# papaboo/Bifrost3D

Measured on AMD Instinct MI355X. Metric: Mrays/sec + ms/frame at 1080p/256spp; per-pixel RMSE vs OptiXRenderer, higher is better.
Workload: dtype f32

## Files before the change

bifrost3d_amd/csrc/hiprenderer.hip:

```cpp
#include "kernels.h"
#ifndef HIPR_WIDE8_LOW_BUCKET
#define HIPR_WIDE8_LOW_BUCKET 0
#endif
#include "wide8_kernels.h"
#include "wide8_refit.h"
#include "launch.h"

#include <hip/hip_runtime.h>

#include <algorithm>
#include <cmath>
#include <cstdarg>
#include <cstdio>
#include <cstdlib>
#include <cstring>
#include <memory>
#include <string>
#include <vector>

using namespace hipr;

namespace {

thread_local std::string g_last_error;

int fail(int status, const char* fmt, ...) {
    char buf[512];
    va_list args;
    va_start(args, fmt);
    vsnprintf(buf, sizeof(buf), fmt, args);
    va_end(args);
    g_last_error = buf;
    fprintf(stderr, "hiprenderer: %s\n", buf);
    return status;
}

#define HIP_TRY(call)                                                                                          \
    do {                                                                                                       \
        hipError_t err__ = (call);                                                                             \
        if (err__ != hipSuccess)                                                                               \
            return fail(err__ == hipErrorOutOfMemory ? HIPR_ERROR_OUT_OF_MEMORY : HIPR_ERROR_HIP, "%s failed: %s (%s:%d)", #call, \
                        hipGetErrorString(err__), __FILE__, __LINE__);                                         \
    } while (0)

struct DeviceBuffer {
    void* ptr = nullptr;
    size_t bytes = 0;
    DeviceBuffer() = default;
    DeviceBuffer(DeviceBuffer&& other) noexcept : ptr(other.ptr), bytes(other.bytes) { other.ptr = nullptr; other.bytes = 0; }
    DeviceBuffer& operator=(DeviceBuffer&& other) noexcept { std::swap(ptr, other.ptr); std::swap(bytes, other.bytes); return *this; }
    ~DeviceBuffer() { release(); }
    int resize(size_t new_bytes) {
        if (new_bytes <= bytes && ptr) return HIPR_OK;
        if (ptr) { (void)hipFree(ptr); ptr = nullptr; bytes = 0; }
        if (new_bytes == 0) return HIPR_OK;
        HIP_TRY(hipMalloc(&ptr, new_bytes));
        bytes = new_bytes;
        return HIPR_OK;
    }
    int upload(const void* src, size_t n, hipStream_t stream) {
        if (n == 0) return HIPR_OK;
        if (int s = resize(n)) return s;
        HIP_TRY(hipMemcpyAsync(ptr, src, n, hipMemcpyHostToDevice, stream));
        return HIPR_OK;
    }
    void release() { if (ptr) (void)hipFree(ptr); ptr = nullptr; bytes = 0; }
    template <typename T> T* as() const { return static_cast<T*>(ptr); }
};

template <typename T, hipError_t (*FREE)(T)>
struct Owned {
    T handle = nullptr;
    Owned() = default;
    Owned(Owned&& other) noexcept : handle(other.handle) { other.handle = nullptr; }
    Owned& operator=(Owned&& other) noexcept { std::swap(handle, other.handle); return *this; }
    ~Owned() { if (handle) (void)FREE(handle); }
    operator T() const { return handle; }
};
hipError_t free_pinned_words(uint32_t* words) { return hipHostFree(words); }
using Stream = Owned<hipStream_t, hipStreamDestroy>;
using Event = Owned<hipEvent_t, hipEventDestroy>;
using PinnedWords = Owned<uint32_t*, free_pinned_words>;
Stream make_stream() { Stream s; if (hipStreamCreateWithFlags(&s.handle, hipStreamNonBlocking) != hipSuccess) s.handle = nullptr; return s; }
Event make_event(unsigned flags = hipEventDisableTiming) { Event e; if (hipEventCreateWithFlags(&e.handle, flags) != hipSuccess) e.handle = nullptr; return e; }
PinnedWords make_pinned_words(size_t count) { PinnedWords p; if (hipHostMalloc((void**)&p.handle, count * sizeof(uint32_t)) != hipSuccess) p.handle = nullptr; return p; }

struct TimedLaunch { int kernel; hipEvent_t start, stop; };

struct Wavefront {
    Stream own_stream;
    hipStream_t stream = nullptr;
    Event shade_done[2], counts_copied[2], finished;
    DeviceBuffer path[2][4], hits, shadow[3], queue_counts, order, order_coat, nee_flags, sort_keys[2], sort_order, sort_temp;
    PinnedWords host_counts;
    uint32_t first_slot = 0, n_slots = 0;

    PathState path_state(int which) const {
        return {path[which][0].as<float4>(), path[which][1].as<float4>(), path[which][2].as<float4>(), path[which][3].as<uint2>()};
    }
    ShadowQueue shadow_queue() const { return {shadow[0].as<float4>(), shadow[1].as<float4>(), shadow[2].as<float4>()}; }
};
constexpr int MAX_WAVEFRONTS = 4;
constexpr int COUNT_PAIR_STRIDE = 16;
constexpr int COUNT_PAIRS = 3, COUNT_LINES = 5;
constexpr int HOST_COUNT_WORDS = 8 + COUNT_LINES * COUNT_PAIR_STRIDE;

struct Preflight {
    uint32_t wide_stack_need = 0;
    uint32_t wide8_height = 0;
};

struct ResidentScene {
    DeviceBuffer nodes, wide_nodes, wide8_slots, triangles, instances, lights;
    DeviceBuffer indices, geometry, texcoords, tints, emissions, materials, textures, texels, environment_PDF, environment_samples;
    DeviceBuffer shade_triangles, trace_triangles, trace_items;
    DeviceBuffer triangle_class;
    DeviceScene args = {};
    Wide8Scene wide8 = {};
    uint32_t wide8_height = 0, wide_stack_entries = 0;
    int stack_size = 16;
    int shading_models = 7;
    bool coverage_textures_r8 = false;
    bool has_environment = true;
    bool has_textures = true;
    bool all_triangles_opaque = false;
    bool any_coated_triangle = false;
    std::vector<HiprMaterial> uploaded_materials;
    std::vector<uint32_t> uploaded_light_types;
    std::vector<HiprInstance> uploaded_instances;
    uint32_t uploaded_texture_count = 0, uploaded_vertex_count = 0, uploaded_index_count = 0;
    uint64_t uploaded_texel_bytes = 0;

    DeviceBuffer refit_leaf_slots, refit_node_slots, refit_exact, refit_moved, refit_partial, refit_scratch;
    std::vector<uint32_t> refit_level_begin;
    uint32_t refit_leaf_count = 0;
    std::vector<uint32_t> refit_node_list, refit_node_words;
    double uploaded_half_area = 0.0, current_half_area = 0.0;
    bool tree_stale = false;

    bool ready = false;
    int chosen_variant = HIPR_TRACE_BVH2;
    void choose_variant(int requested) {
        const bool large = args.node_count > 64;
        int v = requested;
        if (v < 0) v = large ? HIPR_TRACE_WIDE8_PERSISTENT : (args.triangle_count <= SMALL_SCENE_TRIANGLES ? HIPR_TRACE_EXHAUSTIVE : HIPR_TRACE_BVH2);
        if (v == HIPR_TRACE_WIDE8_PERSISTENT && wide8.slot_count == 0) v = HIPR_TRACE_WIDE_PERSISTENT;
        if (v == HIPR_TRACE_WIDE_PERSISTENT && args.wide_node_count == 0) v = HIPR_TRACE_BVH2;
        if (v == HIPR_TRACE_EXHAUSTIVE && args.trace_item_count == 0 && args.triangle_count != 0) v = HIPR_TRACE_BVH2;
        chosen_variant = v;
    }

    int upload(const HiprSceneDesc* s, const Preflight& checked, int requested_variant, bool cull_backfaces, hipStream_t stream);
    int update_geometry(const HiprSceneDesc* s, const Preflight& checked, int requested_variant, bool cull_backfaces, hipStream_t stream);
    int refit_transforms(const HiprInstanceTransform* moved, uint32_t moved_count, const HiprLight* new_lights, uint32_t light_count, hipStream_t stream, HiprRefitResult* out);
    int lights_keep_their_types(const char* who, const HiprLight* new_lights, uint32_t count) const;
// ... 109 lines not shown
        for (Chain& ch : chains) if (ch.stream == on) return ch;
        for (Chain& ch : chains) if (!ch.event) { ch.stream = on; return ch; }
        chains[0] = {on, nullptr};
        return chains[0];
    }
    void break_chain(hipStream_t on) { chain_of(on).event = nullptr; }
    void begin_timed(int kernel, hipStream_t on) {
        if (!timing) return;
        Chain& ch = chain_of(on);
        TimedLaunch t = {kernel, ch.event ? ch.event : next_event(), next_event()};
        if (!t.start || !t.stop) return;
        if (!ch.event) (void)hipEventRecord(t.start, on);
        ch.event = nullptr;
        timed.push_back(t);
    }
    hipEvent_t end_timed(hipStream_t on) {
        if (!timing || timed.empty()) return nullptr;
        (void)hipEventRecord(timed.back().stop, on);
        chain_of(on).event = timed.back().stop;
        return timed.back().stop;
    }
    void collect_times() {
        for (const TimedLaunch& t : timed) {
            float ms = 0;
            if (hipEventElapsedTime(&ms, t.start, t.stop) == hipSuccess) {
                times.milliseconds[t.kernel] += ms;
                times.launches[t.kernel] += 1;
            }
        }
        timed.clear();
        events_used = 0;
        for (Chain& ch : chains) ch.event = nullptr;
    }
};

namespace {

uint32_t grid_for(uint32_t items, uint32_t block, uint32_t max_blocks) {
    uint32_t blocks = (items + block - 1) / block;
    blocks = std::max(1u, std::min(blocks, max_blocks));
    return (blocks + 7u) & ~7u;
}

constexpr uint32_t PAIRING_LIMIT = SMALL_SCENE_TRIANGLES;
void build_trace_items(const HiprTriangle* triangles, uint32_t count, std::vector<float>& items) {
    auto corner = [&](uint32_t t, int k) -> const float* { const HiprTriangle& tri = triangles[t]; return k % 3 == 0 ? tri.v0 : (k % 3 == 1 ? tri.v1 : tri.v2); };
    auto same = [](const float* p, const float* q) { return std::memcmp(p, q, 12) == 0; };
    auto bits = [](uint32_t v) { float f; std::memcpy(&f, &v, 4); return f; };
    std::vector<bool> merged(count, false);
    items.clear();
    for (uint32_t i = 0; i < count; ++i) {
        if (merged[i]) continue;
        int ra = 0, rb = 0;
        uint32_t partner = UINT32_MAX;
        for (uint32_t j = i + 1; count <= PAIRING_LIMIT && j < count && partner == UINT32_MAX; ++j) {
            if (merged[j] || triangles[j].instance_index != triangles[i].instance_index || triangles[j].flags != triangles[i].flags) continue;
            for (int x = 0; x < 3 && partner == UINT32_MAX; ++x)
                for (int y = 0; y < 3 && partner == UINT32_MAX; ++y) {
                    const float *a = corner(i, x), *b = corner(i, x + 1), *c = corner(i, x + 2), *a2 = corner(j, y), *c2 = corner(j, y + 1), *d = corner(j, y + 2);
                    if (!same(a, a2) || !same(c, c2)) continue;
                    float longest = 0.0f, off = 0.0f;
                    for (int k = 0; k < 3; ++k) {
                        longest = std::fmax(longest, std::fmax(std::fabs(b[k] - a[k]), std::fabs(d[k] - a[k])));
                        off = std::fmax(off, std::fabs(d[k] - (a[k] + (c[k] - b[k]))));
                    }
                    if (off <= 1e-6f * longest) { partner = j; ra = x; rb = y; }
                }
        }
        const float *a = corner(i, ra), *b = corner(i, ra + 1), *d = partner == UINT32_MAX ? corner(i, ra + 2) : corner(partner, rb + 2);
        const uint32_t selectors = partner == UINT32_MAX ? 0u : uint32_t((4 - ra) % 3) | uint32_t((5 - ra) % 3) << 2 | uint32_t((4 - rb) % 3) << 4 | uint32_t((5 - rb) % 3) << 6;
        const float item[16] = {a[0], a[1], a[2], b[0] - a[0], b[1] - a[1], b[2] - a[2], d[0] - a[0], d[1] - a[1], d[2] - a[2],
                                bits(triangles[i].instance_index), bits(triangles[i].primitive_index), bits(triangles[i].flags | (partner == UINT32_MAX ? 0u : HIPR_ITEM_QUAD)),
                                bits(i), bits(partner == UINT32_MAX ? i : partner), bits(partner == UINT32_MAX ? triangles[i].primitive_index : triangles[partner].primitive_index),
                                bits(selectors)};
        items.insert(items.end(), item, item + 16);
        if (partner != UINT32_MAX) merged[partner] = true;
    }
}

constexpr uint32_t WORK_SETS = 256;
constexpr uint32_t WORK_SET_WORDS = TRACE_SHARDS * TRACE_SHARD_STRIDE;
constexpr uint32_t WORK_COUNTERS = WORK_SETS * WORK_SET_WORDS;

uint32_t* next_work_counter(HiprContext* c) {
    uint32_t& index = c->pass_slots[c->active_slot].work_index;
    uint32_t* ring = c->work_counters.as<uint32_t>() + size_t(c->active_slot) * WORK_COUNTERS;
    if (index >= WORK_SETS) {
        for (int g = 0; g < MAX_WAVEFRONTS; ++g) if (c->wavefronts[g].stream) (void)hipStreamSynchronize(c->wavefronts[g].stream);
        (void)hipMemsetAsync(ring, 0, WORK_COUNTERS * sizeof(uint32_t), c->stream);
        (void)hipStreamSynchronize(c->stream);
        index = 0;
    }
    return ring + size_t(index++) * WORK_SET_WORDS;
}

template <int STACK, int MODE, bool INSTRUMENT, bool OVERFLOW>
void launch_persistent(HiprContext* c, const Wavefront& w, const PathState& in, const uint32_t* closest_count, const uint32_t* shadow_count, uint32_t upper_bound, int bucket) {
    int& per_cu = c->persistent_blocks_per_cu[MODE][bucket];
    if (per_cu == 0) {
        int blocks = 0;
        if (hipOccupancyMaxActiveBlocksPerMultiprocessor(&blocks, k_trace_persistent<STACK, MODE, INSTRUMENT, OVERFLOW>, TRACE_BLOCK, 0) != hipSuccess || blocks <= 0) blocks = 4;
        if (c->trace_log) fprintf(stderr, "[hipr] k_trace_persistent<%d, %d>: occupancy query says %d blocks of %d threads per CU\n", STACK, MODE, blocks, TRACE_BLOCK);
        if (c->blocks_per_cu_override > 0) blocks = c->blocks_per_cu_override;
        per_cu = blocks;
    }
    const uint32_t waves_per_block = TRACE_BLOCK / 64;
    uint32_t grid = uint32_t(c->cu_count) * uint32_t(per_cu);
    grid = std::max(1u, std::min(grid, (upper_bound + 63u) / 64u / waves_per_block + 1u));
    hipLaunchKernelGGL((k_trace_persistent<STACK, MODE, INSTRUMENT, OVERFLOW>), dim3(grid), dim3(TRACE_BLOCK), 0, w.stream, c->scene.args, in, w.hits.as<float4>(), w.shadow_queue(),
                       c->radiance.as<float4>(), closest_count, shadow_count, next_work_counter(c), c->refill_below, c->counters.as<DeviceCounters>());
}

template <int STACK, int MODE, bool INSTRUMENT>
void launch_wide8(HiprContext* c, const Wavefront& w, const PathState& in, const uint32_t* closest_count, const uint32_t* shadow_count, uint32_t upper_bound, int bucket, const uint32_t* sorted = nullptr) {
    int& per_cu = c->wide8_blocks_per_cu[MODE][bucket];
    if (per_cu == 0) {
        int blocks = 0;
        if (hipOccupancyMaxActiveBlocksPerMultiprocessor(&blocks, k_trace_wide8<STACK, MODE, INSTRUMENT>, TRACE_BLOCK, 0) != hipSuccess || blocks <= 0) blocks = 4;
        if (c->trace_log) fprintf(stderr, "[hipr] k_trace_wide8<%d, %d>: occupancy query says %d blocks of %d threads per CU\n", STACK, MODE, blocks, TRACE_BLOCK);
        if (c->blocks_per_cu_override > 0) blocks = c->blocks_per_cu_override;
        per_cu = blocks;
    }
    const uint32_t waves_per_block = TRACE_BLOCK / 64;
    uint32_t grid = uint32_t(c->cu_count) * uint32_t(c->pipelining_now && per_cu > 2 ? per_cu - c->pipeline_spare_blocks : per_cu);
    grid = std::max(1u, std::min(grid, (upper_bound + 63u) / 64u / waves_per_block + 1u));
#if HIPR_RAY_SORT
    if constexpr (MODE == TRACE_FUSED && !INSTRUMENT) if (sorted) {
        if (c->scene.all_triangles_opaque && c->lean_trace)
            hipLaunchKernelGGL((k_trace_wide8<STACK, MODE, INSTRUMENT, false, true>), dim3(grid), dim3(TRACE_BLOCK), 0, w.stream, c->scene.args, c->scene.wide8, in, w.hits.as<float4>(), w.shadow_queue(),
                               c->radiance.as<float4>(), closest_count, shadow_count, next_work_counter(c), c->refill_below, c->counters.as<DeviceCounters>(), sorted);
        else
            hipLaunchKernelGGL((k_trace_wide8<STACK, MODE, INSTRUMENT, true, true>), dim3(grid), dim3(TRACE_BLOCK), 0, w.stream, c->scene.args, c->scene.wide8, in, w.hits.as<float4>(), w.shadow_queue(),
                               c->radiance.as<float4>(), closest_count, shadow_count, next_work_counter(c), c->refill_below, c->counters.as<DeviceCounters>(), sorted);
        return;
    }
#endif
    if constexpr (!INSTRUMENT && MODE != TRACE_CLOSEST) if (!sorted && !c->scene.all_triangles_opaque && c->scene.coverage_textures_r8 && c->lean_trace) {
        hipLaunchKernelGGL((k_trace_wide8<STACK, MODE, INSTRUMENT, true, false, true>), dim3(grid), dim3(TRACE_BLOCK), 0, w.stream, c->scene.args, c->scene.wide8, in, w.hits.as<float4>(), w.shadow_queue(),
                           c->radiance.as<float4>(), closest_count, shadow_count, next_work_counter(c), c->refill_below, c->counters.as<DeviceCounters>());
        return;
    }
    if (!INSTRUMENT && MODE != TRACE_CLOSEST && c->scene.all_triangles_opaque && c->lean_trace)
        hipLaunchKernelGGL((k_trace_wide8<STACK, MODE, INSTRUMENT, false>), dim3(grid), dim3(TRACE_BLOCK), 0, w.stream, c->scene.args, c->scene.wide8, in, w.hits.as<float4>(), w.shadow_queue(),
                           c->radiance.as<float4>(), closest_count, shadow_count, next_work_counter(c), c->refill_below, c->counters.as<DeviceCounters>());
    else
    hipLaunchKernelGGL((k_trace_wide8<STACK, MODE, INSTRUMENT>), dim3(grid), dim3(TRACE_BLOCK), 0, w.stream, c->scene.args, c->scene.wide8, in, w.hits.as<float4>(), w.shadow_queue(),
                       c->radiance.as<float4>(), closest_count, shadow_count, next_work_counter(c), c->refill_below, c->counters.as<DeviceCounters>());
}

template <int MODE, bool INSTRUMENT>
void launch_persistent_for_stack(HiprContext* c, const Wavefront& w, const PathState& in, const uint32_t* closest_count, const uint32_t* shadow_count, uint32_t upper_bound, const uint32_t* sorted = nullptr) {
    if (c->use_wide8()) {
#if HIPR_WIDE8_LOW_BUCKET
        if (c->scene.wide8_height <= 9u) launch_wide8<8, MODE, INSTRUMENT>(c, w, in, closest_count, shadow_count, upper_bound, 3, sorted);
        else
#endif
        if (c->scene.wide8_height <= uint32_t(WIDE8_STACK_SHALLOW) + 1u) launch_wide8<WIDE8_STACK_SHALLOW, MODE, INSTRUMENT>(c, w, in, closest_count, shadow_count, upper_bound, 0, sorted);
        else if (c->scene.wide8_height <= 17u) launch_wide8<16, MODE, INSTRUMENT>(c, w, in, closest_count, shadow_count, upper_bound, 1, sorted);
        else launch_wide8<32, MODE, INSTRUMENT>(c, w, in, closest_count, shadow_count, upper_bound, 2, sorted);
        return;
    }
#ifndef HIPR_STACK_MID
#define HIPR_STACK_MID 16
#endif
    if (c->scene.wide_stack_entries <= 16) launch_persistent<16, MODE, INSTRUMENT, false>(c, w, in, closest_count, shadow_count, upper_bound, 0);
    else if (c->scene.wide_stack_entries <= 32) launch_persistent<HIPR_STACK_MID, MODE, INSTRUMENT, true>(c, w, in, closest_count, shadow_count, upper_bound, 1);
    else launch_persistent<32, MODE, INSTRUMENT, true>(c, w, in, closest_count, shadow_count, upper_bound, 2);
}

template <bool INSTRUMENT>
void launch_trace_closest(HiprContext* c, const Wavefront& w, const PathState& in, const uint32_t* count_ptr, uint32_t upper_bound) {
    float4* hits = w.hits.as<float4>();
    if (c->use_persistent()) { launch_persistent_for_stack<TRACE_CLOSEST, INSTRUMENT>(c, w, in, count_ptr, nullptr, upper_bound); return; }
    DeviceCounters* dc = c->counters.as<DeviceCounters>();
    if (c->use_exhaustive()) {
        hipLaunchKernelGGL((k_trace_closest_small<INSTRUMENT>), dim3(grid_for(upper_bound, 256, 256u * 16u)), dim3(256), 0, w.stream, c->scene.args, in, hits, count_ptr, dc);
        return;
    }
    const uint32_t grid = grid_for(upper_bound, TRACE_BLOCK, 256u * 16u);
    switch (c->scene.stack_size) {
    case 16: hipLaunchKernelGGL((k_trace_closest<16, INSTRUMENT>), dim3(grid), dim3(TRACE_BLOCK), 0, w.stream, c->scene.args, in, hits, count_ptr, dc); break;
    case 32: hipLaunchKernelGGL((k_trace_closest<32, INSTRUMENT>), dim3(grid), dim3(TRACE_BLOCK), 0, w.stream, c->scene.args, in, hits, count_ptr, dc); break;
    default: hipLaunchKernelGGL((k_trace_closest<64, INSTRUMENT>), dim3(grid), dim3(TRACE_BLOCK), 0, w.stream, c->scene.args, in, hits, count_ptr, dc); break;
    }
}

template <bool INSTRUMENT>
void launch_trace_shadow(HiprContext* c, const Wavefront& w, const uint32_t* count_ptr, uint32_t upper_bound) {
    if (c->use_persistent()) { launch_persistent_for_stack<TRACE_SHADOW, INSTRUMENT>(c, w, PathState{}, nullptr, count_ptr, upper_bound); return; }
    DeviceCounters* dc = c->counters.as<DeviceCounters>();
    float4* rad = c->radiance.as<float4>();
    ShadowQueue q = w.shadow_queue();
    if (c->use_exhaustive()) {
        hipLaunchKernelGGL((k_trace_shadow_small<INSTRUMENT>), dim3(grid_for(upper_bound, 256, 256u * 16u)), dim3(256), 0, w.stream, c->scene.args, q, rad, count_ptr, dc);
        return;
    }
    const uint32_t grid = grid_for(upper_bound, TRACE_BLOCK, 256u * 16u);
    switch (c->scene.stack_size) {
    case 16: hipLaunchKernelGGL((k_trace_shadow<16, INSTRUMENT>), dim3(grid), dim3(TRACE_BLOCK), 0, w.stream, c->scene.args, q, rad, count_ptr, dc); break;
    case 32: hipLaunchKernelGGL((k_trace_shadow<32, INSTRUMENT>), dim3(grid), dim3(TRACE_BLOCK), 0, w.stream, c->scene.args, q, rad, count_ptr, dc); break;
    default: hipLaunchKernelGGL((k_trace_shadow<64, INSTRUMENT>), dim3(grid), dim3(TRACE_BLOCK), 0, w.stream, c->scene.args, q, rad, count_ptr, dc); break;
    }
}

template <bool INSTRUMENT>
void launch_trace_fused(HiprContext* c, const Wavefront& w, const PathState& in, const uint32_t* closest_count, const uint32_t* shadow_count, uint32_t upper_bound) {
    const uint32_t* sorted = nullptr;
#if HIPR_RAY_SORT
    if (!INSTRUMENT && c->coherence_sort && c->use_wide8() && w.sort_order.ptr) {
        const ShadowQueue q = w.shadow_queue();
        hipr::RaySortLaunch a = {w.stream, in.o_tmin, in.d_pdf, q.o_tmax, q.d_slot, closest_count, shadow_count, std::min(upper_bound, 2u * std::max(w.n_slots, 64u)), {}, {},
                                 w.sort_keys[0].as<uint16_t>(), w.sort_keys[1].as<uint16_t>(), w.sort_order.as<uint32_t>(), w.sort_temp.ptr, w.sort_temp.bytes};
        for (int k = 0; k < 3; ++k) { a.grid_min[k] = c->scene.wide8.grid_min[k]; a.cells_per_unit[k] = 16.0f / (c->scene.wide8.grid_cell[k] * 2097152.0f); }
        if (hipr::launch_ray_sort(a) == 0) sorted = w.sort_order.as<uint32_t>();
    }
#endif
    launch_persistent_for_stack<TRACE_FUSED, INSTRUMENT>(c, w, in, closest_count, shadow_count, upper_bound, sorted);
}

void launch_shade(HiprContext* c, const Wavefront& w, const HiprCameraState& camera, int cur, uint32_t alive, const uint32_t* in_count, uint32_t* out_counts, uint32_t* zero_pair, bool camera_rays) {
    const uint32_t* order = nullptr;
    const unsigned long long* listed = nullptr;
    uint32_t* taken_words = w.queue_counts.as<uint32_t>() + COUNT_PAIR_STRIDE * COUNT_PAIRS;
    if (c->shade_ordered && c->use_persistent() && c->entry == HIPR_ENTRY_PATH_TRACING && alive >= c->shade_ordered_from && (!camera_rays || c->shade_ordered_camera)) {
        unsigned long long* taken = reinterpret_cast<unsigned long long*>(taken_words + COUNT_PAIR_STRIDE * cur);
        if (c->shade_classes && c->scene.any_coated_triangle)
            hipLaunchKernelGGL(k_classify_hits<true>, dim3(grid_for(alive, 256u * CLASSIFY_ROUNDS, uint32_t(c->cu_count) * 8u)), dim3(256), 0, w.stream, w.hits.as<float4>(), in_count, w.order.as<uint32_t>(), taken,
                               c->scene.triangle_class.as<unsigned char>(), w.order_coat.as<uint32_t>());
        else
            hipLaunchKernelGGL(k_classify_hits<false>, dim3(grid_for(alive, 256u * CLASSIFY_ROUNDS, uint32_t(c->cu_count) * 8u)), dim3(256), 0, w.stream, w.hits.as<float4>(), in_count, w.order.as<uint32_t>(), taken,
                               (const unsigned char*)nullptr, w.order_coat.as<uint32_t>());
        order = w.order.as<uint32_t>();
        listed = taken;
    }
    const bool split = c->shade_split && c->entry == HIPR_ENTRY_PATH_TRACING && c->scene.args.light_count != 0 && w.nee_flags.ptr;
    const uint32_t blocks_per_cu = c->shade_blocks_per_cu > 0 ? uint32_t(c->shade_blocks_per_cu) : (split ? uint32_t(HIPR_SHADE_SPLIT_WAVES) : (c->scene.shading_models == 2 ? 2u : uint32_t(c->shade_unit().waves_per_simd)));
    PathState shaded = w.path_state(cur);
    if (camera_rays) shaded.thr_bounces = nullptr;
    ShadeLaunch a = {grid_for(alive, SHADE_BLOCK, uint32_t(c->cu_count) * blocks_per_cu), w.stream, c->scene.args, camera, c->frame, c->entry, shaded, w.hits.as<float4>(), order, w.order_coat.as<uint32_t>(), listed, w.path_state(1 - cur),
                     w.shadow_queue(), c->radiance.as<float4>(), in_count, reinterpret_cast<unsigned long long*>(out_counts), reinterpret_cast<unsigned long long*>(zero_pair),
                     reinterpret_cast<unsigned long long*>(taken_words + COUNT_PAIR_STRIDE * (1 - cur)), split ? w.nee_flags.as<unsigned char>() : nullptr,
                     c->counters.as<DeviceCounters>(), c->scene.has_textures || !c->lean_shade, c->scene.has_environment || !c->lean_shade};
    c->shade_unit().shade(c->scene.shading_models, a);
}

int partition_path_slots(HiprContext* c) {
    const FrameInfo& fi = c->frame;
    const uint64_t slots = uint64_t(fi.owned_tiles) * 64u * fi.samples_per_pass;
    c->n_slots = uint32_t(slots);
    c->traced_samples = 0;
    int r = 0;
    c->partitioned_for = c->wavefronts_wanted(true);
    c->wavefront_count = int(std::max<uint64_t>(1, std::min<uint64_t>(uint64_t(c->partitioned_for), slots / 65536u)));
    const uint64_t groups = slots / 64u;
    for (int g = 0; g < MAX_WAVEFRONTS; ++g) {
        Wavefront& w = c->wavefronts[g];
        w.first_slot = uint32_t(g);
        w.n_slots = g >= c->wavefront_count ? 0u : uint32_t((groups + uint64_t(c->wavefront_count) - 1u - uint64_t(g)) / uint64_t(c->wavefront_count) * 64u);
        const bool second_slot = g == 1 && c->wavefront_count == 1 && c->pipeline_passes && c->partitioned_for == 1;
        if (second_slot) { w.first_slot = c->wavefronts[0].first_slot; w.n_slots = c->wavefronts[0].n_slots; }
        const size_t bytes = size_t(std::max(w.n_slots, 64u)) * 16;
        if (g >= c->wavefront_count && !second_slot) {
            for (auto& buffers : w.path) for (DeviceBuffer& b : buffers) b.release();
            w.hits.release(); w.order.release(); w.order_coat.release(); w.nee_flags.release();
            w.sort_keys[0].release(); w.sort_keys[1].release(); w.sort_order.release(); w.sort_temp.release();
            for (DeviceBuffer& b : w.shadow) b.release();
            continue;
        }
        for (int i = 0; i < 2; ++i) for (int j = 0; j < 4; ++j) r |= w.path[i][j].resize(j == 3 ? bytes / 2 : bytes);
        r |= w.hits.resize(bytes);
        r |= w.order.resize(bytes / 4);
        r |= w.order_coat.resize(bytes / 4);
        if (c->shade_split) r |= w.nee_flags.resize(bytes / 16);
#if HIPR_RAY_SORT
        if (c->coherence_sort) {
            const size_t entries = bytes / 16 * 2;
            r |= w.sort_keys[0].resize(entries * 2); r |= w.sort_keys[1].resize(entries * 2); r |= w.sort_order.resize(entries * 4);
            r |= w.sort_temp.resize(hipr::ray_sort_temp_bytes(uint32_t(entries)));
        }
#endif
        for (int j = 0; j < 3; ++j) r |= w.shadow[j].resize(bytes);
    }
    const bool two_slots = c->wavefront_count == 1 && c->pipeline_passes && c->partitioned_for == 1;
    if (!two_slots) {
        if (c->traced_slot == 1 && c->radiance_other.ptr) std::swap(c->radiance, c->radiance_other);
        c->radiance_other.release();
        c->traced_slot = c->next_slot = c->active_slot = 0;
    }
    r |= c->radiance.resize(slots * 16);
    if (two_slots) r |= c->radiance_other.resize(slots * 16);
    return r;
}

void set_frame_divisors(FrameInfo& f) { f.by_samples_per_pass = make_divisor(f.samples_per_pass); f.by_tiles_x = make_divisor(f.tiles_x); }

int check_context(HiprContext* c) {
    if (!c) return fail(HIPR_ERROR_INVALID_ARGUMENT, "null context");
    HIP_TRY(hipSetDevice(c->device));
    return HIPR_OK;
}

int enqueue_bounce(HiprContext* c, Wavefront& w, const HiprCameraState& camera, uint32_t k, uint32_t bound, uint32_t* host_sizes = nullptr) {
    const bool fused = c->use_persistent();
    if (!host_sizes) host_sizes = w.host_counts + 2 * (k & 1u);

    uint32_t* counts = w.queue_counts.as<uint32_t>();
    const int parity = int(k & 1u);
// ... 1429 lines not shown
```

bifrost3d_amd/csrc/wide8_kernels.h:

```cpp
#pragma once

#include "kernels.h"

namespace hipr {

struct Wide8Scene {
    const uint4* slots;
    uint32_t slot_count;
    float grid_min[3], grid_cell[3];
    uint32_t cull_backfaces;
};

constexpr int WIDE8_STACK_SHALLOW = 12;
#ifndef HIPR_WIDE8_WAVES
#define HIPR_WIDE8_WAVES 6
#endif
#ifndef HIPR_WIDE8_SIGN_HITS
#define HIPR_WIDE8_SIGN_HITS 1
#endif
#ifndef HIPR_WIDE8_LEAF_VOTE_NUM
#define HIPR_WIDE8_LEAF_VOTE_NUM 1
#define HIPR_WIDE8_LEAF_VOTE_DEN 2
#endif
#ifndef HIPR_WIDE8_WAVES_LOW
#define HIPR_WIDE8_WAVES_LOW 6
#endif
HD constexpr int wide8_waves_per_simd(int stack_entries) { return stack_entries <= 8 ? HIPR_WIDE8_WAVES_LOW : (stack_entries <= 12 ? HIPR_WIDE8_WAVES : (stack_entries <= 16 ? 5 : 4)); }

template <int STACK, int MODE, bool INSTRUMENT, bool COVERAGE = true, bool SORTED = false, bool COVERAGE_R8 = false>
__global__ __launch_bounds__(TRACE_BLOCK) __attribute__((amdgpu_waves_per_eu(wide8_waves_per_simd(STACK)))) void k_trace_wide8(DeviceScene sc, Wide8Scene tree, PathState in, float4* hits, ShadowQueue q,
        float4* radiance, const uint32_t* closest_count_ptr, const uint32_t* shadow_count_ptr, uint32_t* work_counter, int refill_below, DeviceCounters* counters,
        const uint32_t* sorted = nullptr) {
    __shared__ uint2 s_stack[STACK * TRACE_BLOCK];
    uint2* stack = s_stack + threadIdx.x;
    const uint32_t n_closest = MODE != TRACE_SHADOW ? *closest_count_ptr : 0u;
    const uint32_t n = n_closest + (MODE != TRACE_CLOSEST ? *shadow_count_ptr : 0u);
    const uint32_t lane = threadIdx.x & 63u;
    const unsigned long long lt = (1ull << lane) - 1ull;
    const uint32_t chunk_size = min(TRACE_CHUNK_MAX, max(64u, (n / (gridDim.x * (TRACE_BLOCK / 64u) * 2u)) & ~63u));

    uint32_t chunk_next = 0, chunk_end = 0;
    uint32_t shard = (blockIdx.x & 7u) * (TRACE_SHARDS / 8u) + ((blockIdx.x >> 3) % (TRACE_SHARDS / 8u));
    bool exhausted = false;

    bool active = false, finished = false;
    bool is_shadow = MODE == TRACE_SHADOW;
    uint32_t ray_index = 0;
    f3 o = {0, 0, 0}, d = {0, 0, 1}, inv = {0, 0, 0}, ood = {0, 0, 0};
    float tmin = 0.0f, tmax = 0.0f;
    float pay_x = 0.0f, pay_y = 0.0f, pay_z = __uint_as_float(HIPR_HIT_MISS);
    uint32_t pay_k = HIPR_NO_TRIANGLE;
    uint32_t octant = 0;
    uint32_t gx = 0, gy = 0;
    uint32_t item = 0;
    bool item_is_leaf = false;
    int sp = 0;
    uint32_t nodes = 0, tris = 0, shadow_nodes = 0, shadow_tris = 0;
    uint32_t diag_node_iterations = 0, diag_node_lanes = 0, diag_triangle_iterations = 0, diag_triangle_lanes = 0, diag_busy_lanes = 0, diag_refills = 0;
    uint32_t diag_pushes = 0, diag_pushes_deep = 0;

    for (;;) {
        if (finished) {
            if (is_shadow) {
                if constexpr (MODE != TRACE_CLOSEST) {
                    float4 acc = radiance[pay_k];
                    acc.x += pay_x; acc.y += pay_y; acc.z += pay_z;
                    radiance[pay_k] = acc;
                }
            } else if constexpr (MODE != TRACE_SHADOW) {
                for (uint32_t li = 0; li < sc.light_count; ++li) {
                    const HiprLight l = load_light_uniform(sc.lights, li);
                    const uint32_t type = l.flags & HIPR_LIGHT_TYPE_MASK;
                    float t = -1e30f;
                    if (type == HIPR_LIGHT_SPHERE) { if (!(l.data[6] > 0.0f)) continue; t = ray_sphere(o, d, L3(l, 3), l.data[6]); }
                    else if (type == HIPR_LIGHT_SPOT) { if (!(l.data[6] > 0.0f)) continue; t = ray_disk(o, d, L3(l, 3), L3(l, 7), l.data[6]); }
                    else continue;
                    if (t > tmin && t < tmax) { tmax = t; pay_x = 0; pay_y = 0; pay_z = __uint_as_float(HIPR_HIT_LIGHT | li); }
                }
                hits[ray_index] = make_float4(tmax, pay_x, pay_y, pay_z);
            }
            finished = false;
        }
        const unsigned long long idle = wave_ballot(!active);
        if (INSTRUMENT && lane == 0 && idle && !exhausted) ++diag_refills;
        if (idle && !exhausted) {
            while (chunk_next >= chunk_end && !exhausted) {
                const uint32_t shard_begin = uint32_t((unsigned long long)n * shard / TRACE_SHARDS);
                const uint32_t shard_end = uint32_t((unsigned long long)n * (shard + 1u) / TRACE_SHARDS);
                uint32_t base = 0;
                if (lane == 0) base = atomicAdd(work_counter + shard * TRACE_SHARD_STRIDE, chunk_size);
                base = __shfl(base, 0);
                if (base < shard_end - shard_begin) { chunk_next = shard_begin + base; chunk_end = min(chunk_next + chunk_size, shard_end); }
                else {
                    const uint32_t my_size = uint32_t((unsigned long long)n * (lane + 1u) / TRACE_SHARDS) - uint32_t((unsigned long long)n * lane / TRACE_SHARDS);
                    const uint32_t claimed = __hip_atomic_load(work_counter + lane * TRACE_SHARD_STRIDE, __ATOMIC_RELAXED, __HIP_MEMORY_SCOPE_AGENT);
                    const unsigned long long open = wave_ballot(claimed < my_size);
                    if (!open) exhausted = true;
                    else {
                        const unsigned long long rotated = shard ? ((open >> shard) | (open << (64u - shard))) : open;
                        shard = (shard + uint32_t(__builtin_ctzll(rotated))) % TRACE_SHARDS;
                    }
                }
            }
            if (chunk_next < chunk_end) {
                const uint32_t idx = chunk_next + __popcll(idle & lt);
                if (!active && idx < chunk_end) {
                    bool dead = false;
                    float4 ro, rdv;
                    if (MODE == TRACE_FUSED) is_shadow = idx >= n_closest;
                    const uint32_t entry = SORTED ? sorted[idx] : idx;
                    if (is_shadow) {
                        if constexpr (MODE != TRACE_CLOSEST) {
                            const uint32_t si = entry - n_closest;
                            ray_index = si;
                            ro = q.o_tmax[si]; rdv = q.d_slot[si];
                            const float4 rr = q.radiance[si];
                            pay_x = rr.x; pay_y = rr.y; pay_z = rr.z;
                            pay_k = __float_as_uint(rdv.w);
                            tmin = 0.0f; tmax = ro.w;
                        }
                    } else if constexpr (MODE != TRACE_SHADOW) {
                        ray_index = entry;
                        const uint2 meta = in.meta[entry];
                        dead = meta.x == HIPR_DEAD_SLOT;
                        pay_k = meta.y;
                        ro = in.o_tmin[entry]; rdv = in.d_pdf[entry];
                        tmin = ro.w; tmax = __builtin_inff();
                        pay_x = pay_y = 0.0f; pay_z = __uint_as_float(HIPR_HIT_MISS);
                    }
                    if (dead) hits[entry] = make_float4(0, 0, 0, __uint_as_float(HIPR_HIT_MISS));
                    else {
                        o = mk3(ro.x, ro.y, ro.z); d = mk3(rdv.x, rdv.y, rdv.z);
                        const f3 sd = {fabsf(d.x) > 1e-20f ? d.x : copysignf(1e-20f, d.x), fabsf(d.y) > 1e-20f ? d.y : copysignf(1e-20f, d.y),
                                       fabsf(d.z) > 1e-20f ? d.z : copysignf(1e-20f, d.z)};
                        inv = {1.0f / sd.x, 1.0f / sd.y, 1.0f / sd.z};
                        ood = o * inv;
                        octant = (inv.x < 0.0f ? 1u : 0u) | (inv.y < 0.0f ? 2u : 0u) | (inv.z < 0.0f ? 4u : 0u);
                        sp = 0;
                        gx = 1u << 24; gy = 1u << 8;
                        item = 0u; item_is_leaf = false;
                        if (tree.slot_count == 0) finished = true;
                        else active = true;
                    }
                }
                chunk_next = min(chunk_next + uint32_t(__popcll(idle)), chunk_end);
            }
        }
        unsigned long long busy = wave_ballot(active);
        if (!busy) {
            if (wave_ballot(finished)) continue;
            if (exhausted) break;
            continue;
        }

        do {
            const bool leaf_mode = active & item_is_leaf;
            const bool node_mode = active & !item_is_leaf;
            const unsigned long long lmask = wave_ballot(leaf_mode), nmask = wave_ballot(node_mode);
            bool advance = false;
            if (INSTRUMENT && lane == 0) {
                const bool leaves = __popcll(lmask) * HIPR_WIDE8_LEAF_VOTE_DEN > __popcll(nmask) * HIPR_WIDE8_LEAF_VOTE_NUM;
                diag_triangle_iterations += leaves; diag_triangle_lanes += leaves ? __popcll(lmask) : 0;
                diag_node_iterations += !leaves; diag_node_lanes += leaves ? 0 : __popcll(nmask);
                diag_busy_lanes += __popcll(lmask | nmask);
            }
            if (__popcll(lmask) * HIPR_WIDE8_LEAF_VOTE_DEN > __popcll(nmask) * HIPR_WIDE8_LEAF_VOTE_NUM) {
                if (leaf_mode) {
                    const uint4* rp = tree.slots + 4 * size_t(item);
                    const uint4 r0 = rp[0], r1 = rp[1], r2 = rp[2], r3 = rp[3];
                    const f3 a = mk3(__uint_as_float(r0.x), __uint_as_float(r0.y), __uint_as_float(r0.z));
                    const f3 e1 = mk3(__uint_as_float(r0.w), __uint_as_float(r1.x), __uint_as_float(r1.y));
                    const f3 e2 = mk3(__uint_as_float(r1.z), __uint_as_float(r1.w), __uint_as_float(r2.x));
                    const f3 e3 = mk3(__uint_as_float(r2.y), __uint_as_float(r2.z), __uint_as_float(r2.w));
                    const uint32_t flags = r3.z;
#ifndef HIPR_WIDE8_CULL_CODE
#define HIPR_WIDE8_CULL_CODE 1
#endif
                    const uint32_t cull = HIPR_WIDE8_CULL_CODE && tree.cull_backfaces != 0u ? flags : 0u;
                    const float refuse_a_below = (cull & 4u) ? -__uint_as_float(r3.w) : -__builtin_inff();
                    const float refuse_b_below = (cull & 8u) ? -__uint_as_float(r3.w) : -__builtin_inff();
                    bool testing = true;
                    advance = true;
#pragma unroll
                    for (int which = 0; which < 2; ++which) {
                        const uint32_t id = which == 0 ? r3.x : r3.y;
                        testing = testing & (id != HIPR_LEAF8_NONE);
                        if (testing) {
                            if (INSTRUMENT) { tris += is_shadow ? 0u : 1u; shadow_tris += is_shadow ? 1u : 0u; }
                            TriangleTest test;
                            const f3 first = which == 0 ? e1 : e2, second = which == 0 ? e2 : e3;
                            const bool hit = triangle_inside(a, first, second, o, d, test);
                            float t = 0.0f, ru = 0.0f, rv = 0.0f;
                            if (wave_any(hit)) triangle_hit_values(test, second, t, ru, rv);
                            const float rw = 1.0f - ru - rv;
                            const uint32_t su = (flags >> (which == 0 ? 8 : 12)) & 3u, sv = (flags >> (which == 0 ? 10 : 14)) & 3u;
                            const float u = su == 0u ? rw : (su == 1u ? ru : rv), v = sv == 0u ? rw : (sv == 1u ? ru : rv);
                            if constexpr (MODE != TRACE_CLOSEST) {
                                if (is_shadow && hit && t > tmin && t < tmax) {
                                    float coverage = 1.0f;
                                    if (COVERAGE && !(flags >> which & 1u)) {
                                        const float4* record = sc.shade_triangles + SHADE_TRIANGLE_QUADS * size_t(id);
                                        const float4 r3 = record[3], r6 = record[6], r7 = record[7];
                                        const float w = 1.0f - u - v;
                                        const f2 uv = mk2(r6.z, r6.w) * u + mk2(r7.x, r7.y) * v + mk2(r6.x, r6.y) * w;
                                        coverage = COVERAGE_R8 ? material_coverage_r8(sc, sc.materials[__float_as_uint(r3.w)], uv) : material_coverage(sc, sc.materials[__float_as_uint(r3.w)], uv);
                                    }
                                    pay_x *= 1.0f - coverage; pay_y *= 1.0f - coverage; pay_z *= 1.0f - coverage;
                                    if (pay_x < 0.0000001f && pay_y < 0.0000001f && pay_z < 0.0000001f) {
                                        pay_x = pay_y = pay_z = 0.0f;
                                        testing = false;
                                        gy = 0u; sp = 0;
                                    }
                                }
                            }
                            if constexpr (MODE != TRACE_SHADOW) {
                                const float facing = which == 0 ? test.det : __uint_as_float(__float_as_uint(test.det) ^ ((flags & 16u) << 27));
                                const bool refused = facing < (which == 0 ? refuse_a_below : refuse_b_below);
                                const bool closer = !is_shadow & hit & !refused & (id != pay_k) & (t > tmin) & ((t < tmax) | ((t == tmax) & (id < __float_as_uint(pay_z))));
                                tmax = closer ? t : tmax; pay_x = closer ? u : pay_x; pay_y = closer ? v : pay_y; pay_z = closer ? __uint_as_float(id) : pay_z;
                            }
                        }
                    }
                }
            } else if (node_mode) {
                const uint4* np = tree.slots + 4 * size_t(item);
                const uint4 w0 = np[0], w1 = np[1], w2 = np[2], w3 = np[3];
                if (INSTRUMENT) { nodes += is_shadow ? 0u : 1u; shadow_nodes += is_shadow ? 1u : 0u; }
                advance = true;
                const uint32_t mx = w0.x & 0x1FFFFFu, my = (w0.x >> 21) | ((w0.y & 0x3FFu) << 11), mz = (w0.y >> 10) & 0x1FFFFFu;
                const float ox = fmaf(float(mx), tree.grid_cell[0], tree.grid_min[0]), oy = fmaf(float(my), tree.grid_cell[1], tree.grid_min[1]),
                            oz = fmaf(float(mz), tree.grid_cell[2], tree.grid_min[2]);
                const float ax = __uint_as_float((w0.z & 0xFFu) << 23) * inv.x, ay = __uint_as_float(((w0.z >> 8) & 0xFFu) << 23) * inv.y,
                            az = __uint_as_float(((w0.z >> 16) & 0xFFu) << 23) * inv.z;
                const float bx = fmaf(ox, inv.x, -ood.x), by = fmaf(oy, inv.y, -ood.y), bz = fmaf(oz, inv.z, -ood.z);
                const bool px = ax >= 0.0f, py = ay >= 0.0f, pz = az >= 0.0f;
                const uint32_t nx[2] = {px ? w1.x : w2.z, px ? w1.y : w2.w}, fx[2] = {px ? w2.z : w1.x, px ? w2.w : w1.y};
                const uint32_t ny[2] = {py ? w1.z : w3.x, py ? w1.w : w3.y}, fy[2] = {py ? w3.x : w1.z, py ? w3.y : w1.w};
                const uint32_t nz[2] = {pz ? w2.x : w3.z, pz ? w2.y : w3.w}, fz[2] = {pz ? w3.z : w2.x, pz ? w3.w : w2.y};
                uint32_t h = 0u;
#if HIPR_WIDE8_SIGN_HITS
#pragma unroll
                for (int k = 7; k >= 0; --k) {
                    const int word = k >> 2, shift = 8 * (k & 3);
                    const float x0 = fmaf(float((nx[word] >> shift) & 0xFFu), ax, bx), x1 = fmaf(float((fx[word] >> shift) & 0xFFu), ax, bx);
                    const float y0 = fmaf(float((ny[word] >> shift) & 0xFFu), ay, by), y1 = fmaf(float((fy[word] >> shift) & 0xFFu), ay, by);
                    const float z0 = fmaf(float((nz[word] >> shift) & 0xFFu), az, bz), z1 = fmaf(float((fz[word] >> shift) & 0xFFu), az, bz);
                    const float tnear = fmaxf(fmaxf(x0, y0), fmaxf(z0, tmin));
                    const float tfar = fminf(fminf(fminf(x1, y1), z1), tmax);
                    h = __builtin_amdgcn_alignbit(h, __float_as_uint(fmaf(tfar, 1.0000004f, -tnear)), 31u);
                }
                h = ~h & (w0.w >> 24);
#else
#pragma unroll
                for (int k = 0; k < 8; ++k) {
                    const int word = k >> 2, shift = 8 * (k & 3);
                    const float x0 = fmaf(float((nx[word] >> shift) & 0xFFu), ax, bx), x1 = fmaf(float((fx[word] >> shift) & 0xFFu), ax, bx);
                    const float y0 = fmaf(float((ny[word] >> shift) & 0xFFu), ay, by), y1 = fmaf(float((fy[word] >> shift) & 0xFFu), ay, by);
                    const float z0 = fmaf(float((nz[word] >> shift) & 0xFFu), az, bz), z1 = fmaf(float((fz[word] >> shift) & 0xFFu), az, bz);
                    const float tnear = fmaxf(fmaxf(x0, y0), fmaxf(z0, tmin));
                    float tfar = fminf(fminf(x1, y1), z1);
                    tfar = fminf(tfar, tmax) * 1.0000004f;
                    h |= tnear <= tfar ? (1u << k) : 0u;
                }
                h &= w0.w >> 24;
#endif
                h = (octant & 1u) ? (((h & 0x55u) << 1) | ((h >> 1) & 0x55u)) : h;
                h = (octant & 2u) ? (((h & 0x33u) << 2) | ((h >> 2) & 0x33u)) : h;
                h = (octant & 4u) ? (((h & 0x0Fu) << 4) | (h >> 4)) : h;
                if (h) {
                    if (gy & 0xFFu) {
                        stack[sp * TRACE_BLOCK] = make_uint2(gx, gy);
                        if (INSTRUMENT) { ++diag_pushes; diag_pushes_deep += sp >= 8; }
                        ++sp;
                    }
                    gx = w0.w;
                    gy = h | (w0.z >> 24) << 8;
                }
            }
            if (advance) {
                if ((gy & 0xFFu) == 0u && sp > 0) {
                    --sp;
                    const uint2 popped = stack[sp * TRACE_BLOCK];
                    gx = popped.x; gy = popped.y;
                }
                const bool done = (gy & 0xFFu) == 0u;
                const uint32_t p = uint32_t(__builtin_ctz(gy | 0x100u));
                gy = done ? gy : (gy & (gy - 1u));
                const uint32_t position = (p ^ octant) & 7u;
                item_is_leaf = !((gy >> (8u + position)) & 1u);
                item = (gx & 0xFFFFFFu) + uint32_t(__popc((gx >> 24) & ((1u << position) - 1u)));
                active = !done;
                finished = done;
            }
            busy = wave_ballot(active);
        } while (busy && (exhausted || __popcll(busy) >= refill_below));
    }

    if (INSTRUMENT) {
        wave_add(&counters->node_iterations, diag_node_iterations); wave_add(&counters->node_lanes, diag_node_lanes);
        wave_add(&counters->triangle_iterations, diag_triangle_iterations); wave_add(&counters->triangle_lanes, diag_triangle_lanes);
        wave_add(&counters->busy_lanes, diag_busy_lanes); wave_add(&counters->refills, diag_refills);
        wave_add(&counters->pushes, diag_pushes); wave_add(&counters->pushes_past_16, diag_pushes_deep);
        if (MODE != TRACE_SHADOW) { wave_add(&counters->closest_nodes, nodes); wave_add(&counters->closest_triangles, tris); }
        if (MODE != TRACE_CLOSEST) { wave_add(&counters->shadow_nodes, shadow_nodes); wave_add(&counters->shadow_triangles, shadow_tris); }
    }
}

}
```

Baseline: 5604.

## Stage ray refills through per-wave LDS ring and enable low-stack wide8 bucket

Enables the low-stack (8-entry) wide8 bucket by default. For that bucket it adds a per-wave shared-memory ring that prefetches up to 64 rays with coalesced loads, so idle lanes refill from LDS instead of scattered global reads. Shadow radiance accumulation is split so the read is issued before the refill and the write after it, and zero-contribution shadow rays skip the read-modify-write entirely. The cost is more LDS per block, which may lower occupancy, plus extra fences and more complex control flow.

```diff
diff --git a/bifrost3d_amd/csrc/hiprenderer.hip b/bifrost3d_amd/csrc/hiprenderer.hip
--- a/bifrost3d_amd/csrc/hiprenderer.hip
+++ b/bifrost3d_amd/csrc/hiprenderer.hip
@@ -1,6 +1,6 @@
 #include "kernels.h"
 #ifndef HIPR_WIDE8_LOW_BUCKET
-#define HIPR_WIDE8_LOW_BUCKET 0
+#define HIPR_WIDE8_LOW_BUCKET 1
 #endif
 #include "wide8_kernels.h"
 #include "wide8_refit.h"
@@ -416,7 +416,7 @@
 void launch_persistent_for_stack(HiprContext* c, const Wavefront& w, const PathState& in, const uint32_t* closest_count, const uint32_t* shadow_count, uint32_t upper_bound, const uint32_t* sorted = nullptr) {
     if (c->use_wide8()) {
 #if HIPR_WIDE8_LOW_BUCKET
-        if (c->scene.wide8_height <= 9u) launch_wide8<8, MODE, INSTRUMENT>(c, w, in, closest_count, shadow_count, upper_bound, 3, sorted);
+        if (c->scene.wide8_height <= uint32_t(WIDE8_STACK_LOW) + 1u) launch_wide8<WIDE8_STACK_LOW, MODE, INSTRUMENT>(c, w, in, closest_count, shadow_count, upper_bound, 3, sorted);
         else
 #endif
         if (c->scene.wide8_height <= uint32_t(WIDE8_STACK_SHALLOW) + 1u) launch_wide8<WIDE8_STACK_SHALLOW, MODE, INSTRUMENT>(c, w, in, closest_count, shadow_count, upper_bound, 0, sorted);
diff --git a/bifrost3d_amd/csrc/wide8_kernels.h b/bifrost3d_amd/csrc/wide8_kernels.h
--- a/bifrost3d_amd/csrc/wide8_kernels.h
+++ b/bifrost3d_amd/csrc/wide8_kernels.h
@@ -25,6 +25,15 @@
 #ifndef HIPR_WIDE8_WAVES_LOW
 #define HIPR_WIDE8_WAVES_LOW 6
 #endif
+constexpr int WIDE8_STACK_LOW = 8;
+#ifndef HIPR_WIDE8_RING
+#define HIPR_WIDE8_RING 1
+#endif
+#ifndef HIPR_WIDE8_RETIRE_AHEAD
+#define HIPR_WIDE8_RETIRE_AHEAD 1
+#endif
+constexpr int WIDE8_RING_WORDS = 9;
+HD constexpr int wide8_ring_rays(int stack_entries) { return HIPR_WIDE8_RING && stack_entries <= WIDE8_STACK_LOW ? 64 : 0; }
 HD constexpr int wide8_waves_per_simd(int stack_entries) { return stack_entries <= 8 ? HIPR_WIDE8_WAVES_LOW : (stack_entries <= 12 ? HIPR_WIDE8_WAVES : (stack_entries <= 16 ? 5 : 4)); }
 
 template <int STACK, int MODE, bool INSTRUMENT, bool COVERAGE = true, bool SORTED = false, bool COVERAGE_R8 = false>
@@ -33,6 +42,11 @@
         const uint32_t* sorted = nullptr) {
     __shared__ uint2 s_stack[STACK * TRACE_BLOCK];
     uint2* stack = s_stack + threadIdx.x;
+    constexpr uint32_t RING = uint32_t(wide8_ring_rays(STACK));
+    static_assert((RING & (RING - 1u)) == 0u, "the ring wraps by masking");
+    __shared__ uint32_t s_ring[RING ? RING * WIDE8_RING_WORDS * (TRACE_BLOCK / 64u) : 1u];
+    uint32_t* ring = s_ring + (threadIdx.x >> 6) * (RING * WIDE8_RING_WORDS);
+    uint32_t ring_head = 0, ring_count = 0;
     const uint32_t n_closest = MODE != TRACE_SHADOW ? *closest_count_ptr : 0u;
     const uint32_t n = n_closest + (MODE != TRACE_CLOSEST ? *shadow_count_ptr : 0u);
     const uint32_t lane = threadIdx.x & 63u;
@@ -60,12 +74,24 @@
     uint32_t diag_pushes = 0, diag_pushes_deep = 0;
 
     for (;;) {
+        bool add_pending = false;
+        float4 add_to = {0, 0, 0, 0};
+        float add_x = 0.0f, add_y = 0.0f, add_z = 0.0f;
+        uint32_t add_slot = 0;
         if (finished) {
             if (is_shadow) {
                 if constexpr (MODE != TRACE_CLOSEST) {
+#if HIPR_WIDE8_RETIRE_AHEAD
+                    if (pay_x != 0.0f || pay_y != 0.0f || pay_z != 0.0f) {
+                        add_pending = true;
+                        add_slot = pay_k; add_x = pay_x; add_y = pay_y; add_z = pay_z;
+                        add_to = radiance[pay_k];
+                    }
+#else
                     float4 acc = radiance[pay_k];
                     acc.x += pay_x; acc.y += pay_y; acc.z += pay_z;
                     radiance[pay_k] = acc;
+#endif
                 }
             } else if constexpr (MODE != TRACE_SHADOW) {
                 for (uint32_t li = 0; li < sc.light_count; ++li) {
@@ -81,75 +107,171 @@
             }
             finished = false;
         }
-        const unsigned long long idle = wave_ballot(!active);
-        if (INSTRUMENT && lane == 0 && idle && !exhausted) ++diag_refills;
-        if (idle && !exhausted) {
-            while (chunk_next >= chunk_end && !exhausted) {
-                const uint32_t shard_begin = uint32_t((unsigned long long)n * shard / TRACE_SHARDS);
-                const uint32_t shard_end = uint32_t((unsigned long long)n * (shard + 1u) / TRACE_SHARDS);
-                uint32_t base = 0;
-                if (lane == 0) base = atomicAdd(work_counter + shard * TRACE_SHARD_STRIDE, chunk_size);
-                base = __shfl(base, 0);
-                if (base < shard_end - shard_begin) { chunk_next = shard_begin + base; chunk_end = min(chunk_next + chunk_size, shard_end); }
+        auto claim_chunk = [&]() {
+        while (chunk_next >= chunk_end && !exhausted) {
+            const uint32_t shard_begin = uint32_t((unsigned long long)n * shard / TRACE_SHARDS);
+            const uint32_t shard_end = uint32_t((unsigned long long)n * (shard + 1u) / TRACE_SHARDS);
+            uint32_t base = 0;
+            if (lane == 0) base = atomicAdd(work_counter + shard * TRACE_SHARD_STRIDE, chunk_size);
+            base = __shfl(base, 0);
+            if (base < shard_end - shard_begin) { chunk_next = shard_begin + base; chunk_end = min(chunk_next + chunk_size, shard_end); }
+            else {
+                const uint32_t my_size = uint32_t((unsigned long long)n * (lane + 1u) / TRACE_SHARDS) - uint32_t((unsigned long long)n * lane / TRACE_SHARDS);
+                const uint32_t claimed = __hip_atomic_load(work_counter + lane * TRACE_SHARD_STRIDE, __ATOMIC_RELAXED, __HIP_MEMORY_SCOPE_AGENT);
+                const unsigned long long open = wave_ballot(claimed < my_size);
+                if (!open) exhausted = true;
                 else {
-                    const uint32_t my_size = uint32_t((unsigned long long)n * (lane + 1u) / TRACE_SHARDS) - uint32_t((unsigned long long)n * lane / TRACE_SHARDS);
-                    const uint32_t claimed = __hip_atomic_load(work_counter + lane * TRACE_SHARD_STRIDE, __ATOMIC_RELAXED, __HIP_MEMORY_SCOPE_AGENT);
-                    const unsigned long long open = wave_ballot(claimed < my_size);
-                    if (!open) exhausted = true;
-                    else {
-                        const unsigned long long rotated = shard ? ((open >> shard) | (open << (64u - shard))) : open;
-                        shard = (shard + uint32_t(__builtin_ctzll(rotated))) % TRACE_SHARDS;
-                    }
-                }
-            }
-            if (chunk_next < chunk_end) {
-                const uint32_t idx = chunk_next + __popcll(idle & lt);
-                if (!active && idx < chunk_end) {
-                    bool dead = false;
-                    float4 ro, rdv;
-                    if (MODE == TRACE_FUSED) is_shadow = idx >= n_closest;
-                    const uint32_t entry = SORTED ? sorted[idx] : idx;
+                    const unsigned long long rotated = shard ? ((open >> shard) | (open << (64u - shard))) : open;
+                    shard = (shard + uint32_t(__builtin_ctzll(rotated))) % TRACE_SHARDS;
+                }
+            }
+        }
+        };
+        if constexpr (RING != 0u) {
+            const unsigned long long idle = wave_ballot(!active);
+            const bool refilling = idle && !(exhausted && ring_count == 0u);
+            if (INSTRUMENT && lane == 0 && refilling) ++diag_refills;
+            if (refilling) {
+                const uint32_t want = uint32_t(__popcll(idle));
+                while (ring_count < want && !exhausted) {
+                    claim_chunk();
+                    if (chunk_next >= chunk_end) break;
+                    const uint32_t take = min(min(RING - ring_count, 64u), chunk_end - chunk_next);
+                    bool stage = false;
+                    float4 ro = {0, 0, 0, 0}, rdv = {0, 0, 0, 0};
+                    uint32_t from = 0, tag = 0;
+                    if (lane < take) {
+                        const uint32_t idx = chunk_next + lane;
+                        const uint32_t entry = SORTED ? sorted[idx] : idx;
+                        if (MODE == TRACE_SHADOW || (MODE == TRACE_FUSED && idx >= n_closest)) {
+                            if constexpr (MODE != TRACE_CLOSEST) {
+                                const uint32_t si = entry - n_closest;
+                                ro = q.o_tmax[si]; rdv = q.d_slot[si];
+                                from = __float_as_uint(rdv.w);
+                                tag = si | 0x80000000u;
+                                stage = true;
+                            }
+                        } else if constexpr (MODE != TRACE_SHADOW) {
+                            const uint2 meta = in.meta[entry];
+                            ro = in.o_tmin[entry]; rdv = in.d_pdf[entry];
+                            from = meta.y;
+                            tag = entry;
+                            stage = meta.x != HIPR_DEAD_SLOT;
+                            if (!stage) {
+                                float zero = 0.0f, miss = __uint_as_float(HIPR_HIT_MISS);
+                                asm volatile("" : "+v"(zero), "+v"(miss));
+                                hits[entry] = make_float4(zero, zero, zero, miss);
+                            }
+                        }
+                    }
+                    const unsigned long long staged = wave_ballot(stage);
+                    if (stage) {
+                        uint32_t* e = ring + ((ring_head + ring_count + uint32_t(__popcll(staged & lt))) & (RING - 1u));
+                        e[0 * RING] = __float_as_uint(ro.x); e[1 * RING] = __float_as_uint(ro.y); e[2 * RING] = __float_as_uint(ro.z); e[3 * RING] = __float_as_uint(ro.w);
+                        e[4 * RING] = __float_as_uint(rdv.x); e[5 * RING] = __float_as_uint(rdv.y); e[6 * RING] = __float_as_uint(rdv.z);
+                        e[7 * RING] = from; e[8 * RING] = tag;
+                    }
+                    ring_count += uint32_t(__popcll(staged));
+                    chunk_next += take;
+                }
+                __builtin_amdgcn_fence(__ATOMIC_ACQ_REL, "wavefront");
+                const uint32_t k = uint32_t(__popcll(idle & lt));
+                if (!active && k < ring_count) {
+                    const uint32_t* e = ring + ((ring_head + k) & (RING - 1u));
+                    o = mk3(__uint_as_float(e[0 * RING]), __uint_as_float(e[1 * RING]), __uint_as_float(e[2 * RING]));
+                    const float t = __uint_as_float(e[3 * RING]);
+                    d = mk3(__uint_as_float(e[4 * RING]), __uint_as_float(e[5 * RING]), __uint_as_float(e[6 * RING]));
+                    pay_k = e[7 * RING];
+                    const uint32_t tag = e[8 * RING];
+                    ray_index = tag & 0x7FFFFFFFu;
+                    if (MODE == TRACE_FUSED) is_shadow = (tag >> 31) != 0u;
                     if (is_shadow) {
                         if constexpr (MODE != TRACE_CLOSEST) {
-                            const uint32_t si = entry - n_closest;
-                            ray_index = si;
-                            ro = q.o_tmax[si]; rdv = q.d_slot[si];
-                            const float4 rr = q.radiance[si];
+                            const float4 rr = q.radiance[ray_index];
                             pay_x = rr.x; pay_y = rr.y; pay_z = rr.z;
-                            pay_k = __float_as_uint(rdv.w);
-                            tmin = 0.0f; tmax = ro.w;
+                            tmin = 0.0f; tmax = t;
                         }
                     } else if constexpr (MODE != TRACE_SHADOW) {
-                        ray_index = entry;
-                        const uint2 meta = in.meta[entry];
-                        dead = meta.x == HIPR_DEAD_SLOT;
-                        pay_k = meta.y;
-                        ro = in.o_tmin[entry]; rdv = in.d_pdf[entry];
-                        tmin = ro.w; tmax = __builtin_inff();
+                        tmin = t; tmax = __builtin_inff();
                         pay_x = pay_y = 0.0f; pay_z = __uint_as_float(HIPR_HIT_MISS);
                     }
-                    if (dead) hits[entry] = make_float4(0, 0, 0, __uint_as_float(HIPR_HIT_MISS));
-                    else {
-                        o = mk3(ro.x, ro.y, ro.z); d = mk3(rdv.x, rdv.y, rdv.z);
-                        const f3 sd = {fabsf(d.x) > 1e-20f ? d.x : copysignf(1e-20f, d.x), fabsf(d.y) > 1e-20f ? d.y : copysignf(1e-20f, d.y),
-                                       fabsf(d.z) > 1e-20f ? d.z : copysignf(1e-20f, d.z)};
-                        inv = {1.0f / sd.x, 1.0f / sd.y, 1.0f / sd.z};
-                        ood = o * inv;
-                        octant = (inv.x < 0.0f ? 1u : 0u) | (inv.y < 0.0f ? 2u : 0u) | (inv.z < 0.0f ? 4u : 0u);
-                        sp = 0;
-                        gx = 1u << 24; gy = 1u << 8;
-                        item = 0u; item_is_leaf = false;
-                        if (tree.slot_count == 0) finished = true;
-                        else active = true;
-                    }
-                }
-                chunk_next = min(chunk_next + uint32_t(__popcll(idle)), chunk_end);
+                    const f3 sd = {fabsf(d.x) > 1e-20f ? d.x : copysignf(1e-20f, d.x), fabsf(d.y) > 1e-20f ? d.y : copysignf(1e-20f, d.y),
+                                   fabsf(d.z) > 1e-20f ? d.z : copysignf(1e-20f, d.z)};
+                    inv = {1.0f / sd.x, 1.0f / sd.y, 1.0f / sd.z};
+                    ood = o * inv;
+                    octant = (inv.x < 0.0f ? 1u : 0u) | (inv.y < 0.0f ? 2u : 0u) | (inv.z < 0.0f ? 4u : 0u);
+                    sp = 0;
+                    gx = 1u << 24; gy = 1u << 8;
+                    item = 0u; item_is_leaf = false;
+                    if (tree.slot_count == 0) finished = true;
+                    else active = true;
+                }
+                const uint32_t taken = min(want, ring_count);
+                ring_head = (ring_head + taken) & (RING - 1u);
+                ring_count -= taken;
+                __builtin_amdgcn_fence(__ATOMIC_ACQ_REL, "wavefront");
+            }
+        } else {
+            const unsigned long long idle = wave_ballot(!active);
+            if (INSTRUMENT && lane == 0 && idle && !exhausted) ++diag_refills;
+            if (idle && !exhausted) {
+                claim_chunk();
+                if (chunk_next < chunk_end) {
+                    const uint32_t idx = chunk_next + __popcll(idle & lt);
+                    if (!active && idx < chunk_end) {
+                        bool dead = false;
+                        float4 ro, rdv;
+                        if (MODE == TRACE_FUSED) is_shadow = idx >= n_closest;
+                        const uint32_t entry = SORTED ? sorted[idx] : idx;
+                        if (is_shadow) {
+                            if constexpr (MODE != TRACE_CLOSEST) {
+                                const uint32_t si = entry - n_closest;
+                                ray_index = si;
+                                ro = q.o_tmax[si]; rdv = q.d_slot[si];
+                                const float4 rr = q.radiance[si];
+                                pay_x = rr.x; pay_y = rr.y; pay_z = rr.z;
+                                pay_k = __float_as_uint(rdv.w);
+                                tmin = 0.0f; tmax = ro.w;
+                            }
+                        } else if constexpr (MODE != TRACE_SHADOW) {
+                            ray_index = entry;
+                            const uint2 meta = in.meta[entry];
+                            dead = meta.x == HIPR_DEAD_SLOT;
+                            pay_k = meta.y;
+                            ro = in.o_tmin[entry]; rdv = in.d_pdf[entry];
+                            tmin = ro.w; tmax = __builtin_inff();
+                            pay_x = pay_y = 0.0f; pay_z = __uint_as_float(HIPR_HIT_MISS);
+                        }
+                        if (dead) hits[entry] = make_float4(0, 0, 0, __uint_as_float(HIPR_HIT_MISS));
+                        else {
+                            o = mk3(ro.x, ro.y, ro.z); d = mk3(rdv.x, rdv.y, rdv.z);
+                            const f3 sd = {fabsf(d.x) > 1e-20f ? d.x : copysignf(1e-20f, d.x), fabsf(d.y) > 1e-20f ? d.y : copysignf(1e-20f, d.y),
+                                           fabsf(d.z) > 1e-20f ? d.z : copysignf(1e-20f, d.z)};
+                            inv = {1.0f / sd.x, 1.0f / sd.y, 1.0f / sd.z};
+                            ood = o * inv;
+                            octant = (inv.x < 0.0f ? 1u : 0u) | (inv.y < 0.0f ? 2u : 0u) | (inv.z < 0.0f ? 4u : 0u);
+                            sp = 0;
+                            gx = 1u << 24; gy = 1u << 8;
+                            item = 0u; item_is_leaf = false;
+                            if (tree.slot_count == 0) finished = true;
+                            else active = true;
+                        }
+                    }
+                    chunk_next = min(chunk_next + uint32_t(__popcll(idle)), chunk_end);
+                }
             }
         }
+        if constexpr (MODE != TRACE_CLOSEST) {
+            if (add_pending) {
+                add_to.x += add_x; add_to.y += add_y; add_to.z += add_z;
+                radiance[add_slot] = add_to;
+            }
+        }
+        const bool drained = exhausted && ring_count == 0u;
         unsigned long long busy = wave_ballot(active);
         if (!busy) {
             if (wave_ballot(finished)) continue;
-            if (exhausted) break;
+            if (drained) break;
             continue;
         }
 
@@ -293,7 +415,7 @@
                 finished = done;
             }
             busy = wave_ballot(active);
-        } while (busy && (exhausted || __popcll(busy) >= refill_below));
+        } while (busy && (drained || __popcll(busy) >= refill_below));
     }
 
     if (INSTRUMENT) {
```

Result: no change. 5654 (median of 6 runs) (+0.9%).
